# DataCTE/SDXL-Training-Improvements

Measured on AMD Instinct MI355X. Metric: images/sec/node SDXL-base 1024^2 bf16 fwd+bwd, higher is better.
Workload: dtype bf16; 1 GPU; method=ddpm v_prediction + zero_terminal_snr + MinSNR(5), SDXL-base UNet fwd+bwd, batch 4/GPU, 1024^2 (latent 128x128); global_batch=4, parallelism=dp1, weights=synthetic (counter-hash init of the 2,567,463,684-parameter SDXL-base UNet)

## Files before the change

sdxl-training-improvements_amd/csrc/gemm.hip:

```cpp
#include "gemm_tiles.h"

#include <stdio.h>
#include <stdlib.h>

#include <type_traits>
#include <vector>

#define BM 128
#ifndef GEMM_DIRECT_EPILOGUE
#define GEMM_DIRECT_EPILOGUE 1
#endif

static int g_mode256 = 1;
static int g_force_cfg = 0;
#ifdef SDXL_DIAG
static int g_sk_mode = 0;
#endif

static constexpr int cdiv_c(int a, int b) { return (a + b - 1) / b; }
__device__ unsigned g_ln_spin_error = 0;
__device__ __forceinline__ float row16_sum(float v) {
  v += __builtin_bit_cast(float, __builtin_amdgcn_update_dpp(0, __builtin_bit_cast(int, v), 0x111, 0xf, 0xf, true));
  v += __builtin_bit_cast(float, __builtin_amdgcn_update_dpp(0, __builtin_bit_cast(int, v), 0x112, 0xf, 0xf, true));
  v += __builtin_bit_cast(float, __builtin_amdgcn_update_dpp(0, __builtin_bit_cast(int, v), 0x114, 0xf, 0xf, true));
  v += __builtin_bit_cast(float, __builtin_amdgcn_update_dpp(0, __builtin_bit_cast(int, v), 0x118, 0xf, 0xf, true));
  return v;
}
__device__ __forceinline__ bf16x8 z8() {
  bf16x8 z;
#pragma unroll
  for (int e = 0; e < 8; ++e) z[e] = (bf16)0.f;
  return z;
}
static constexpr int gemm_smem_bytes(int BN, int S, int BK, int NW = 4) {
  const bool pad = ((BM * BK * 2 / 1024) % NW) != 0 || ((BN * BK * 2 / 1024) % NW) != 0;
  int ring = S * (BM + BN) * BK * 2 + (pad ? 1024 : 0), stg = BK == 32 ? 0 : 64 * (BN + 4) * 4;
  return ring > stg ? ring : stg;
}
static constexpr int gemm_occupancy(int BN, int S, int BK, int NW) {
  int byl = (160 * 1024) / gemm_smem_bytes(BN, S, BK, NW);
  return NW == 8 ? 1 : (byl > 3 ? 3 : (byl < 1 ? 1 : byl));
}

template <int FORM, bool CONV, int BN, int S, int BK, bool FAST, int NW, bool KSP = false, bool PL = false>
__global__ __launch_bounds__(NW * 64, PL ? 2 : gemm_occupancy(BN, S, BK, NW)) void gemm_kernel(const GemmP pin) {
  GemmP p = pin;
  set_wave_prio(pin.prio);
  int bx, by, bz = blockIdx.z, ztap = 0;
  if (FORM == GEMM_TN && pin.xcd_bh > 0) {
    const int tz = pin.group > 1 ? 1 : (int)gridDim.z / pin.splitk;
    xcd_seq_map(pin.xcd_bh, tz, bx, by, ztap, bz);
  } else xcd_tile_map(pin.xcd_px, bx, by);
  if (FORM == GEMM_TN && pin.group > 1) {
    const int gi = bz;
    p.A = pin.gA[gi]; p.B = pin.gB[gi]; p.C = pin.gC[gi]; p.bias_grad = pin.gbias_grad[gi]; p.Cb = pin.gCb[gi];
  }
  static_assert(!KSP || (NW == 8 && BK == 64 && FAST && S >= 3 && FORM != GEMM_TN), "split-K groups: 8 waves, BK 64, FAST staging, ring >= 3");
  static_assert(!PL || (NW == 4 && BK == 64 && FAST && S >= 3 && FORM != GEMM_TN && !KSP), "pipelined loop: 4 waves, BK 64, FAST staging, ring >= 3, NT / NN");
  constexpr int BMT = BM;
  constexpr int A_TILE_BYTES = BMT * BK * 2;
  constexpr int B_TILE_BYTES = BN * BK * 2;
  constexpr int STAGE_BYTES = A_TILE_BYTES + B_TILE_BYTES;
  constexpr int RING_BYTES = S * STAGE_BYTES;
  constexpr int WGM = KSP ? 2 : NW / 2;
  constexpr int MI = BMT / (WGM * 16);
  constexpr int NJ = BN / 32;
  constexpr int NCA = A_TILE_BYTES / 1024;
  constexpr int NCB = B_TILE_BYTES / 1024;
  constexpr int ACH = cdiv_c(NCA, NW);
  constexpr int BCH = cdiv_c(NCB, NW);
  constexpr int NL = ACH + BCH;
  constexpr int VR = BK / 8;
  constexpr int KC_ROWS = 64 / VR;
  constexpr int LDC = BN + 4;
  constexpr int NT = NW * 64;
  constexpr bool PIPE = true;
  constexpr bool DIRECT = GEMM_DIRECT_EPILOGUE;
  extern __shared__ __attribute__((aligned(16))) char smem[];
  const int tid = threadIdx.x;
  const int lane = tid & 63;
  const int wave = __builtin_amdgcn_readfirstlane(tid >> 6);
  const int kg = KSP ? wave >> 2 : 0;
  const int wm = KSP ? (wave >> 1) & 1 : wave >> 1, wn = wave & 1;
  const int l16 = lane & 15, g = lane >> 4;
#ifdef SDXL_GEMM_DIAG
  constexpr int dbg = SDXL_GEMM_DIAG;
#else
  constexpr int dbg = 0;
#endif
  const int n0 = (dbg & 8) ? 0 : bx * BN;
  const int m0 = (dbg & 8) ? 0 : by * BMT;

  int tap_fixed = 0, split = 0;
  if (FORM == GEMM_TN && p.group <= 1) {
    if (pin.xcd_bh > 0) {
      split = bz;
      tap_fixed = ztap;
    } else {
      tap_fixed = bz / p.splitk;
      split = bz - tap_fixed * p.splitk;
    }
  }
  constexpr bool NSPLIT = FORM != GEMM_TN && FAST && !KSP;
  if (NSPLIT && p.splitk > 1) split = bz;
  const int ktiles_per_tap = (p.K + BK - 1) / BK;
  int kt_begin = 0, kt_end;
  if (FORM == GEMM_TN) {
    int chunk = (ktiles_per_tap + p.splitk - 1) / p.splitk;
    kt_begin = split * chunk;
    kt_end = min(ktiles_per_tap, kt_begin + chunk);
  } else if (NSPLIT && p.splitk > 1) {
    const int total = ktiles_per_tap * p.taps;
    int chunk = (total + p.splitk - 1) / p.splitk;
    kt_begin = split * chunk;
    kt_end = min(total, kt_begin + chunk);
  } else {
    kt_end = ktiles_per_tap * p.taps;
  }
  const int dn_phase = (FORM == GEMM_NN && CONV && p.up2 == 2) ? m0 / p.up_plane : 0;
  const int dn_nb = (dn_phase & 1) ? 2 : 1;
  if (FORM == GEMM_NN && CONV && p.up2 == 2) kt_end = ktiles_per_tap * ((dn_phase >> 1) ? 2 : 1) * dn_nb;

  const int kc_rowl = lane / VR, kc_pv = lane % VR;
  PixRow arow[ACH];
  if (CONV && !FAST && FORM != GEMM_TN) {
#pragma unroll
    for (int j = 0; j < ACH; ++j) arow[j] = decode_pix(m0 + (wave + j * NW) * KC_ROWS + kc_rowl, p.M, p.Hm, p.Wm);
  }
  const bf16* zsrc = (const bf16*)g_zero16;
  char* const pad_dst = smem + RING_BYTES;

  constexpr bool CF = FAST && CONV;
  const bf16* pa[ACH];
  const bf16* pb[BCH];
  long sa[ACH], sb[BCH];
  int amask[ACH];
  int bok[BCH];
  int by_[BCH], bx_[BCH];
  long ua = 0, ub = 0;
  int s_tap = 0, s_c = 0;
  const int tdy = (SDXL_UP2_3 && p.up2 == 3) ? (tap_fixed / 3 == 0 ? -1 : 0) : p.up2 ? up2_dy(tap_fixed) : tap_fixed / 3 - 1;
  const int tdx = (SDXL_UP2_3 && p.up2 == 3) ? (tap_fixed % 3 == 0 ? -1 : 0) : p.up2 ? up2_dx(tap_fixed) : tap_fixed - (tap_fixed / 3) * 3 - 1;
  const long s3_plane = (SDXL_UP2_3 && p.up2 == 3) ? (long)(((tap_fixed / 3 != 1) ? 2 : 0) + ((tap_fixed % 3 != 1) ? 1 : 0)) * p.up_plane : 0;
  const int up_phase = (CF && FORM == GEMM_NT && p.up2) ? m0 / p.up_plane : dn_phase;
  auto tap_offsets = [&]() {
    int dy, dx, wtap;
    long plane = 0;
    if (FORM == GEMM_NT && (SDXL_UP2_3 && p.up2 == 3)) {
      const int ky = s_tap / 3, kx = s_tap - ky * 3;
      dy = ky == 0 ? -1 : 0; dx = kx == 0 ? -1 : 0;
      wtap = s_tap;
      plane = (long)((ky != 1 ? 2 : 0) + (kx != 1 ? 1 : 0)) * p.up_plane * p.lda;
    } else
    if (FORM == GEMM_NN && p.up2 == 2) {
      const int a = dn_phase >> 1, b = dn_phase & 1;
      const int ry = s_tap / dn_nb, rx = s_tap - ry * dn_nb;
      const int ky = a ? (ry == 0 ? 0 : 2) : 1, kx = b ? (rx == 0 ? 0 : 2) : 1;
      dy = a ? (ry == 0 ? 1 : 0) : 0; dx = b ? (rx == 0 ? 1 : 0) : 0;
      wtap = ky * 3 + kx;
    } else
    if (p.up2) {
      const int e = FORM == GEMM_NT ? up_phase * 4 + s_tap : s_tap;
      dy = up2_dy(e); dx = up2_dx(e); wtap = e;
// ... 130 lines not shown
  auto advance = [&]() {
    if (!CF) return;
    if (FORM == GEMM_TN) {
      ua += (long)BK * p.lda;
      ub += (long)BK * p.ldb;
      const int dxs = BK % p.Wm, dys = BK / p.Wm;
#pragma unroll
      for (int j = 0; j < BCH; ++j) {
        bx_[j] += dxs;
        if (bx_[j] >= p.Wm) { bx_[j] -= p.Wm; by_[j] += 1; }
        by_[j] += dys;
        if (by_[j] >= p.Hm) by_[j] -= p.Hm;
      }
    } else {
      if (++s_c == ktiles_per_tap) { s_c = 0; ++s_tap; }
      tap_offsets();
    }
  };
  bool dma_on = true;
  auto issue_piece = [&](int pc, int buf, bool live) {
    if (dbg && !dma_on) return;
    char* At = smem + buf * STAGE_BYTES;
    char* Bt = At + A_TILE_BYTES;
#pragma unroll
    for (int j = 0; j < ACH; ++j)
      if (pc == j) {
        const int c = wave + j * NW;
        const bf16* src;
        if (CF) {
          const bool v = live && (FORM == GEMM_TN ? amask[j] != 0 : ((amask[j] >> s_tap) & 1) != 0);
          src = v ? pa[j] + ua : zsrc;
        } else {
          src = live ? pa[j] : zsrc;
        }
        char* dst = (NCA % NW == 0 || c < NCA) ? At + c * 1024 : pad_dst;
        if (PL) lds_dma16_global(src, lds_addr_of(dst));
        else __builtin_amdgcn_global_load_lds((gbl_void*)src, (lds_void*)dst, 16, 0, 0);
        if (!CF) pa[j] += sa[j];
      }
#pragma unroll
    for (int j = 0; j < BCH; ++j)
      if (pc == ACH + j) {
        const int c = wave + j * NW;
        const bf16* src;
        if (CF) {
          bool v = live && bok[j] != 0;
          if (FORM == GEMM_TN) {
            const int ys = by_[j] + tdy, xs = bx_[j] + tdx;
            v = v && ys >= 0 && ys < p.Hm && xs >= 0 && xs < p.Wm;
          }
          src = v ? pb[j] + ub : zsrc;
        } else {
          src = live ? pb[j] : zsrc;
        }
        char* dst = (NCB % NW == 0 || c < NCB) ? Bt + c * 1024 : pad_dst;
        if (PL) lds_dma16_global(src, lds_addr_of(dst));
        else __builtin_amdgcn_global_load_lds((gbl_void*)src, (lds_void*)dst, 16, 0, 0);
        if (!CF) pb[j] += sb[j];
      }
  };

  auto stage_gen = [&](int kt, int buf) {
    int tap = 0, c0;
    if (FORM == GEMM_TN) {
      tap = tap_fixed;
      c0 = kt * BK;
    } else {
      tap = kt / ktiles_per_tap;
      c0 = (kt - tap * ktiles_per_tap) * BK;
    }
    const int dy = tap / 3, dx = tap - dy * 3;
    char* At = smem + buf * STAGE_BYTES;
    char* Bt = At + A_TILE_BYTES;
#pragma unroll
    for (int j = 0; j < ACH; ++j) {
      const int c = wave + j * NW;
      const bool cok = NCA % NW == 0 || c < NCA;
      const bf16* src;
      if (FORM == GEMM_TN) {
        const int krow = c * 4 + (lane >> 4);
        const int kk = c0 + krow;
        const int m = m0 + (nc_logical<128>(krow, lane & 15) << 3);
        src = (cok && kk < p.K && m < p.M) ? p.A + (long)kk * p.lda + m : zsrc;
      } else {
        const int row = c * KC_ROWS + kc_rowl;
        const int kofs = c0 + ((kc_pv ^ kc_swz<BK>(row)) << 3);
        if (CONV) {
          long s = gather_src(arow[j], dy, dx, p);
          src = (cok && s >= 0 && kofs < p.K) ? p.A + s * p.lda + kofs : zsrc;
        } else {
          const int m = m0 + row;
          src = (cok && m < p.M && kofs < p.K) ? p.A + (long)m * p.lda + kofs : zsrc;
        }
      }
      __builtin_amdgcn_global_load_lds((gbl_void*)src, (lds_void*)(cok ? At + c * 1024 : pad_dst), 16, 0, 0);
    }
#pragma unroll
    for (int j = 0; j < BCH; ++j) {
      const int c = wave + j * NW;
      const bool cok = NCB % NW == 0 || c < NCB;
      const bf16* src;
      if (FORM == GEMM_NT) {
        const int wtap = p.flip ? (p.taps - 1 - tap) : tap;
        const int row = c * KC_ROWS + kc_rowl;
        const int n = n0 + row;
        const int kofs = c0 + ((kc_pv ^ kc_swz<BK>(row)) << 3);
        src = (cok && n < p.N && kofs < p.K) ? p.B + (long)n * p.ldb + (long)wtap * p.b_tap_stride + kofs : zsrc;
      } else {
        constexpr int V = BN / 8;
        const int q = c * 64 + lane;
        const int krow = q / V, pv = q - krow * V;
        const int kk = c0 + krow;
        const int n = n0 + (nc_logical<BN>(krow, pv) << 3);
        if (FORM == GEMM_NN) {
          const int wtap = p.flip ? (p.taps - 1 - tap) : tap;
          src = (cok && kk < p.K && n < p.N) ? p.B + (long)kk * p.ldb + (long)wtap * p.b_tap_stride + n : zsrc;
        } else {
          long s;
          if (CONV) {
            PixRow r = decode_pix(kk, p.K, p.Hm, p.Wm);
            s = gather_src(r, dy, dx, p);
          } else {
            s = kk < p.K ? kk : -1;
          }
          src = (cok && s >= 0 && n < p.N) ? p.B + s * p.ldb + n : zsrc;
        }
      }
      __builtin_amdgcn_global_load_lds((gbl_void*)src, (lds_void*)(cok ? Bt + c * 1024 : pad_dst), 16, 0, 0);
    }
  };
  auto stage = [&](int kt, int buf) {
    if (FAST) {
#pragma unroll
      for (int pc = 0; pc < NL; ++pc) issue_piece(pc, buf, true);
      advance();
    } else {
      stage_gen(kt, buf);
    }
  };

  f32x4 acc[MI][NJ];
#pragma unroll
  for (int i = 0; i < MI; ++i)
#pragma unroll
    for (int j = 0; j < NJ; ++j) acc[i][j] = (f32x4){0.f, 0.f, 0.f, 0.f};
  const bool do_bias = FORM == GEMM_TN && p.bias_grad != nullptr && bx == 0 && (p.up2 == 1 ? (tap_fixed & 3) == 0 : tap_fixed == 0) && wn == 0;
  f32x4 accb[MI];
  bf16x8 ones;
#pragma unroll
  for (int i = 0; i < MI; ++i) accb[i] = (f32x4){0.f, 0.f, 0.f, 0.f};
#pragma unroll
  for (int e = 0; e < 8; ++e) ones[e] = (bf16)1.0f;

  const int T = kt_end - kt_begin;
  constexpr int U = 1;
#pragma unroll
  for (int d = 0; d < S - U; ++d) {
    if (d < T) stage(kt_begin + d, d);
    else if (FAST) {
#pragma unroll
      for (int pc = 0; pc < NL; ++pc) issue_piece(pc, d, false);
      advance();
    }
  }
  int rd = 0, wr = S - U;
  if (dbg & 2) dma_on = false;
  constexpr int KS = BK / 32;
  struct FragK { bf16x8 a[MI], b[NJ]; };
  auto read_ks = [&](int slot, int ks, FragK& f) {
    const char* At = smem + slot * STAGE_BYTES;
    const char* Bt = At + A_TILE_BYTES;
    if (dbg & 4) {
#pragma unroll
      for (int i = 0; i < MI; ++i) f.a[i] = ones;
#pragma unroll
      for (int j = 0; j < NJ; ++j) f.b[j] = ones;
      return;
    }
#pragma unroll
    for (int i = 0; i < MI; ++i) {
      if (FORM == GEMM_TN)
        f.a[i] = frag_nc<128>(At, ks * 32 + g * 8, wm * (MI * 16) + i * 16, l16);
      else
        f.a[i] = frag_kc<BK>(At, wm * (MI * 16) + i * 16 + l16, ks * 4 + g);
      if (i == 0) {
#pragma unroll
        for (int j = 0; j < NJ; ++j) {
          if (FORM == GEMM_NT)
            f.b[j] = frag_kc<BK>(Bt, wn * (BN / 2) + j * 16 + l16, ks * 4 + g);
          else
            f.b[j] = frag_nc<BN>(Bt, ks * 32 + g * 8, wn * (BN / 2) + j * 16, l16);
        }
      }
    }
  };
  auto mfma_ks = [&](const FragK& f, int ks, int wslot, bool live) {
    if (FORM == GEMM_TN && do_bias) {
#pragma unroll
      for (int i = 0; i < MI; ++i) accb[i] = __builtin_amdgcn_mfma_f32_16x16x32_bf16(f.a[i], ones, accb[i], 0, 0, 0);
    }
    if (!FAST) __builtin_amdgcn_s_setprio(1);
#pragma unroll
    for (int i = 0; i < MI; ++i) {
#pragma unroll
      for (int j = 0; j < NJ; ++j) {
        if (dbg & 1) acc[i][j][0] += (float)f.a[i][0] + (float)f.b[j][0];
        else if (DIRECT) acc[i][j] = __builtin_amdgcn_mfma_f32_16x16x32_bf16(f.b[j], f.a[i], acc[i][j], 0, 0, 0);
        else acc[i][j] = __builtin_amdgcn_mfma_f32_16x16x32_bf16(f.a[i], f.b[j], acc[i][j], 0, 0, 0);
      }
      if (FAST) {
        constexpr int NSLOT = KSP ? MI : KS * MI;
        const int slot = KSP ? i : ks * MI + i;
#pragma unroll
        for (int pc = 0; pc < NL; ++pc)
          if (pc % NSLOT == slot) issue_piece(pc, wslot, live);
      }
    }
    if (!FAST) __builtin_amdgcn_s_setprio(0);
  };
  if constexpr (PL) {
    constexpr int NG = MI;
    constexpr int NITEM = MI + NJ;
    constexpr int RG = 3;
    auto np0 = []() constexpr { int n = 0; for (int pc = 0; pc < NL; ++pc) if (pc % (2 * NG) < NG) ++n; return n; };
    auto read_item = [&](int slot, int ks, FragK& f, int it) {
      const char* At = smem + slot * STAGE_BYTES;
      const char* Bt = At + A_TILE_BYTES;
      if (dbg & 4) { if (it < NJ) f.b[it] = ones; else f.a[it - NJ] = ones; return; }
      if (it < NJ) {
        const int j = it;
        if (FORM == GEMM_NT) f.b[j] = frag_kc<BK>(Bt, wn * (BN / 2) + j * 16 + l16, ks * 4 + g);
        else f.b[j] = frag_nc<BN>(Bt, ks * 32 + g * 8, wn * (BN / 2) + j * 16, l16);
      } else {
        const int i = it - NJ;
        f.a[i] = frag_kc<BK>(At, wm * (MI * 16) + i * 16 + l16, ks * 4 + g);
      }
    };
    auto phase = [&](auto PHC, const FragK& fc, FragK& fn, int rslot, int rks, int wslot, bool live) {
      constexpr int PH = decltype(PHC)::value;
#pragma unroll
      for (int gi = 0; gi < NG; ++gi) {
#pragma unroll
        for (int j = 0; j < NJ; ++j) {
          if (dbg & 1) acc[gi][j][0] += (float)fc.a[gi][0] + (float)fc.b[j][0];
          else acc[gi][j] = __builtin_amdgcn_mfma_f32_16x16x32_bf16(fc.b[j], fc.a[gi], acc[gi][j], 0, 0, 0);
        }
        __builtin_amdgcn_sched_barrier(0);
        if (gi < RG) {
#pragma unroll
          for (int it = 0; it < NITEM; ++it)
            if (it * RG / NITEM == gi) read_item(rslot, rks, fn, it);
        }
#pragma unroll
        for (int pc = 0; pc < NL; ++pc)
          if (pc % (2 * NG) == PH * NG + gi) issue_piece(pc, wslot, live);
        __builtin_amdgcn_sched_barrier(0);
      }
    };
    FragK f0, f1;
    wait_vmcnt<(S - 2) * NL>();
    __builtin_amdgcn_s_barrier();
#pragma unroll
    for (int it = 0; it < NITEM; ++it) read_item(rd, 0, f0, it);
    for (int t = 0; t < T; ++t) {
      const bool live = t + S - 1 < T;
      phase(std::integral_constant<int, 0>{}, f0, f1, rd, 1, wr, live);
      wait_vmcnt<(S - 3) * NL + np0()>();
      asm volatile("s_waitcnt lgkmcnt(0)" ::: "memory");
      __builtin_amdgcn_sched_barrier(0);
      __builtin_amdgcn_s_barrier();
      const int rn = rd + 1 == S ? 0 : rd + 1;
      phase(std::integral_constant<int, 1>{}, f1, f0, rn, 0, wr, live);
      advance();
      rd = rn;
      wr = wr + 1 == S ? 0 : wr + 1;
    }
  } else
  if (KSP) {
    wait_vmcnt<(S - 2) * NL>();
    __builtin_amdgcn_s_barrier();
    if (kg == 1) __builtin_amdgcn_s_barrier();
    for (int t = 0; t < T; ++t) {
      FragK f;
      read_ks(rd, kg, f);
      wait_vmcnt<(S - 3) * NL>();
      __builtin_amdgcn_sched_barrier(0);
      __builtin_amdgcn_s_barrier();
      __builtin_amdgcn_s_setprio(1);
      mfma_ks(f, kg, wr, t + S - 1 < T);
      __builtin_amdgcn_s_setprio(0);
      advance();
      __builtin_amdgcn_sched_barrier(0);
      __builtin_amdgcn_s_barrier();
      rd = rd + 1 == S ? 0 : rd + 1;
      wr = wr + 1 == S ? 0 : wr + 1;
    }
    if (kg == 0) __builtin_amdgcn_s_barrier();
  } else
  for (int t = 0; t < T; ++t) {
    if (FAST) wait_vmcnt<(S - 2) * NL>();
    else if (S >= 3 && t + S - 2 < T) wait_vmcnt<(S - 2) * NL>();
    else wait_vmcnt<0>();
    __builtin_amdgcn_s_barrier();
    const bool live = t + S - 1 < T;
    if (!FAST && live) stage(kt_begin + t + S - 1, wr);
    FragK f[KS];
#pragma unroll
    for (int ks = 0; ks < KS; ++ks) read_ks(rd, ks, f[ks]);
    if (PIPE) __builtin_amdgcn_sched_barrier(0);
#pragma unroll
    for (int ks = 0; ks < KS; ++ks) mfma_ks(f[ks], ks, wr, live);
    if (FAST) advance();
    rd = rd + 1 == S ? 0 : rd + 1;
    wr = wr + 1 == S ? 0 : wr + 1;
  }
  wait_vmcnt<0>();
  if (KSP) {
    __syncthreads();
    float* X = (float*)smem;
#pragma unroll
    for (int i = 0; i < MI; ++i) {
      if ((i >> 1) == kg) continue;
#pragma unroll
      for (int j = 0; j < NJ; ++j)
        *(f32x4*)(X + (wm * 64 + i * 16 + l16) * LDC + wn * (BN / 2) + j * 16 + g * 4) = acc[i][j];
    }
    __syncthreads();
#pragma unroll
    for (int i = 0; i < MI; ++i) {
      if ((i >> 1) != kg) continue;
#pragma unroll
      for (int j = 0; j < NJ; ++j) {
        const f32x4 o = *(const f32x4*)(X + (wm * 64 + i * 16 + l16) * LDC + wn * (BN / 2) + j * 16 + g * 4);
        acc[i][j][0] += o[0]; acc[i][j][1] += o[1]; acc[i][j][2] += o[2]; acc[i][j][3] += o[3];
      }
    }
  }
  if (FORM == GEMM_TN && do_bias && l16 == 0) {
#pragma unroll
    for (int i = 0; i < MI; ++i)
#pragma unroll
      for (int r = 0; r < 4; ++r) {
        const int m = m0 + wm * (MI * 16) + i * 16 + g * 4 + r;
        if (m < p.M) {
          if (p.up2 == 1) atomicAdd(p.bias_grad + m, accb[i][r]);
          else gemm_bias_out(p.bias_grad, p.slab, p.slab_ld, p.splitk, split, p.M, m, accb[i][r]);
        }
      }
  }
  auto store_bf16 = [&](int m, int n, float (&x)[8], int cnt) {
    if (m >= p.M || n >= p.N) return;
    if (cnt == 8) {
      if (p.bias) {
        bf16x8 bv = *(const bf16x8*)(p.bias + n);
#pragma unroll
        for (int e = 0; e < 8; ++e) x[e] += (float)bv[e];
      }
      if (p.rowvec) {
        bf16x8 tv = *(const bf16x8*)(p.rowvec + (long)(m / p.rows_per_batch) * p.ldv + n);
#pragma unroll
        for (int e = 0; e < 8; ++e) x[e] += (float)tv[e];
      }
      if (p.resid) {
        bf16x8 rv = *(const bf16x8*)(p.resid + (long)m * p.ldr + n);
#pragma unroll
        for (int e = 0; e < 8; ++e) x[e] += (float)rv[e];
      }
      bf16x8 o;
#pragma unroll
      for (int e = 0; e < 8; ++e) o[e] = (bf16)x[e];
      *(bf16x8*)((bf16*)p.C + (long)m * p.ldc + n) = o;
    } else {
      if (p.bias) {
        bf16x4 bv = *(const bf16x4*)(p.bias + n);
#pragma unroll
        for (int e = 0; e < 4; ++e) x[e] += (float)bv[e];
      }
      if (p.rowvec) {
        bf16x4 tv = *(const bf16x4*)(p.rowvec + (long)(m / p.rows_per_batch) * p.ldv + n);
#pragma unroll
        for (int e = 0; e < 4; ++e) x[e] += (float)tv[e];
      }
      if (p.resid) {
        bf16x4 rv = *(const bf16x4*)(p.resid + (long)m * p.ldr + n);
#pragma unroll
        for (int e = 0; e < 4; ++e) x[e] += (float)rv[e];
      }
      bf16x4 o;
#pragma unroll
      for (int e = 0; e < 4; ++e) o[e] = (bf16)x[e];
      *(bf16x4*)((bf16*)p.C + (long)m * p.ldc + n) = o;
    }
  };
  if (NSPLIT && p.splitk > 1) {
#pragma unroll
    for (int i = 0; i < MI; ++i) {
      const int m = m0 + wm * (MI * 16) + i * 16 + l16;
      if (m >= p.M) continue;
#pragma unroll
      for (int j = 0; j < NJ; ++j) {
        const int n = n0 + wn * (BN / 2) + j * 16 + g * 4;
        if (n >= p.N) continue;
        *(f32x4*)(p.slab + ((long)split * p.M + m) * p.slab_ld + n) = acc[i][j];
      }
    }
    return;
  }
  constexpr bool LN_OK = SDXL_LN_EPILOGUE && FORM == GEMM_NN && !CONV && BN == 128 && NW == 4 && !KSP && FAST && BK == 64 && S == 2;
  if constexpr (LN_OK) if (p.ln_x) {
    constexpr int NP = NJ / 2;
    asm volatile("s_nop 7\n\ts_nop 7\n\ts_nop 7" ::: "memory");
    __syncthreads();
    float* rowpart = (float*)smem;
    float* rowtot = rowpart + 2 * 128 * 2;
    float* colpart = rowtot + 2 * 128 * 2;
    const int wcol = n0 + wn * (BN / 2);
    const int mrow = m0 + wm * (MI * 16) + l16;
    float s1[MI], s2[MI], mean[MI], rstd[MI];
#pragma unroll
    for (int i = 0; i < MI; ++i) {
      const bool mok = mrow + i * 16 < p.M;
      mean[i] = mok ? p.ln_stats[(long)(mrow + i * 16) * 2] : 0.f;
      rstd[i] = mok ? p.ln_stats[(long)(mrow + i * 16) * 2 + 1] : 0.f;
      s1[i] = 0.f; s2[i] = 0.f;
    }
#pragma unroll
    for (int jp = 0; jp < NP; ++jp) {
      const int j = 2 * jp;
      const int nc = wcol + (j + (g & 1)) * 16 + (g >> 1) * 8;
      const bool nok = nc < p.N;
      bf16x8 gv = z8();
      if (nok) gv = *(const bf16x8*)(p.ln_gamma + nc);
      float pg[8], pb[8];
#pragma unroll
      for (int e = 0; e < 8; ++e) { pg[e] = 0.f; pb[e] = 0.f; }
#pragma unroll
      for (int i = 0; i < MI; ++i) {
        const int m = mrow + i * 16;
        const bool ok = nok && m < p.M;
        float v[8];
#pragma unroll
        for (int r = 0; r < 4; ++r) {
          float lo = acc[i][j][r], hi = acc[i][j + 1][r];
          asm volatile("s_nop 1\n\tv_permlane16_swap_b32 %0, %1" : "+v"(lo), "+v"(hi));
          lo = (float)(bf16)lo; hi = (float)(bf16)hi;
          acc[i][j][r] = lo; acc[i][j + 1][r] = hi;
          v[r] = lo; v[4 + r] = hi;
        }
        if (p.C && ok) {
          bf16x8 o;
#pragma unroll
          for (int e = 0; e < 8; ++e) o[e] = (bf16)v[e];
          *(bf16x8*)((bf16*)p.C + (long)m * p.ldc + nc) = o;
        }
        bf16x8 xv = z8();
        if (ok) xv = *(const bf16x8*)(p.ln_x + (long)m * p.ln_ldx + nc);
#pragma unroll
        for (int e = 0; e < 8; ++e) {
          const float xh = ((float)xv[e] - mean[i]) * rstd[i];
          const float t = v[e] * (float)gv[e];
          s1[i] += t; s2[i] += t * xh;
          pg[e] += v[e] * xh; pb[e] += v[e];
        }
        __builtin_amdgcn_sched_barrier(0);
      }
      if (p.ln_pcol) {
#pragma unroll
        for (int e = 0; e < 8; ++e) {
// ... 45 lines not shown
    __syncthreads();
    if (tid == 0) __hip_atomic_store(flags + (long)bx * gridDim.y + by, (unsigned)p.ln_epoch, __ATOMIC_RELAXED, __HIP_MEMORY_SCOPE_AGENT);
    if (tid < 64) {
      int spins = 0;
      bool ok;
      do {
        unsigned f = (unsigned)p.ln_epoch;
        if (tid < ncolt) f = __hip_atomic_load(flags + (long)tid * gridDim.y + by, __ATOMIC_RELAXED, __HIP_MEMORY_SCOPE_AGENT);
        ok = __all(f == (unsigned)p.ln_epoch);
        if (!ok) __builtin_amdgcn_s_sleep(4);
      } while (!ok && ++spins < (1 << 22));
      if (!ok && tid == 0) atomicOr(&g_ln_spin_error, 1u);
    }
    __syncthreads();
    {
      constexpr int KC = 5;
      const int row = tid & (BMT - 1), h = tid >> 7;
      u64 a[KC], b[KC];
      int spins = 0;
      bool ok;
      do {
#pragma unroll
        for (int k = 0; k < KC; ++k) {
          const int c = 2 * k + h;
          a[k] = tag; b[k] = tag;
          if (c < ncolt) {
            const u64* src = slots + ((long)c * Mpad + m0 + row) * 2;
            a[k] = __hip_atomic_load(src, __ATOMIC_RELAXED, __HIP_MEMORY_SCOPE_AGENT);
            b[k] = __hip_atomic_load(src + 1, __ATOMIC_RELAXED, __HIP_MEMORY_SCOPE_AGENT);
          }
        }
        ok = true;
#pragma unroll
        for (int k = 0; k < KC; ++k) ok = ok && (a[k] >> 32) == (tag >> 32) && (b[k] >> 32) == (tag >> 32);
        if (!ok) __builtin_amdgcn_s_sleep(8);
      } while (!ok && ++spins < (1 << 20));
      if (!ok) atomicOr(&g_ln_spin_error, 2u);
      float S1 = 0.f, S2 = 0.f;
#pragma unroll
      for (int k = 0; k < KC; ++k)
        if (2 * k + h < ncolt) { S1 += __uint_as_float((unsigned)a[k]); S2 += __uint_as_float((unsigned)b[k]); }
      rowtot[(h * BMT + row) * 2] = S1;
      rowtot[(h * BMT + row) * 2 + 1] = S2;
    }
    __syncthreads();
    float S1[MI], S2[MI];
#pragma unroll
    for (int i = 0; i < MI; ++i) {
      const int row = wm * (MI * 16) + i * 16 + l16;
      const float invn = 1.f / (float)p.N;
      S1[i] = (rowtot[row * 2] + rowtot[(BMT + row) * 2]) * invn; S2[i] = (rowtot[row * 2 + 1] + rowtot[(BMT + row) * 2 + 1]) * invn;
    }
#pragma unroll
    for (int jp = 0; jp < NP; ++jp) {
      const int j = 2 * jp;
      const int nc = wcol + (j + (g & 1)) * 16 + (g >> 1) * 8;
      if (nc >= p.N) continue;
      const bf16x8 gv = *(const bf16x8*)(p.ln_gamma + nc);
#pragma unroll
      for (int i = 0; i < MI; ++i) {
        const int m = mrow + i * 16;
        if (m >= p.M) continue;
        const bf16x8 xv = *(const bf16x8*)(p.ln_x + (long)m * p.ln_ldx + nc);
        bf16x8 o;
        if (p.ln_addend) o = *(const bf16x8*)(p.ln_addend + (long)m * p.ln_ldo + nc);
#pragma unroll
        for (int e = 0; e < 8; ++e) {
          const float v = e < 4 ? acc[i][j][e & 3] : acc[i][j + 1][e & 3];
          const float xh = ((float)xv[e] - mean[i]) * rstd[i];
          float d = rstd[i] * (v * (float)gv[e] - S1[i] - xh * S2[i]);
          if (p.ln_addend) d += (float)o[e];
          o[e] = (bf16)d;
        }
        *(bf16x8*)(p.ln_dx + (long)m * p.ln_ldo + nc) = o;
        __builtin_amdgcn_sched_barrier(0);
      }
    }
    return;
  }
  if (FORM == GEMM_TN || !p.geglu) {
    if (FORM != GEMM_TN) asm volatile("s_nop 7\n\ts_nop 7\n\ts_nop 7" ::: "memory");
#pragma unroll
    for (int i = 0; i < MI; ++i) {
      if (KSP && (i >> 1) != kg) continue;
      const int m = m0 + wm * (MI * 16) + i * 16 + l16;
      if (FORM == GEMM_TN) {
        if (m >= p.M) continue;
#pragma unroll
        for (int j = 0; j < NJ; ++j) {
          const int n = n0 + wn * (BN / 2) + j * 16 + g * 4;
          if (n >= p.N) continue;
          f32x4 x = acc[i][j];
          float* c = (float*)p.C + (long)m * p.ldc + (long)tap_fixed * p.c_tap_stride + n;
          if (p.splitk > 1) {
            *(f32x4*)(p.slab + ((long)split * p.M + m) * p.slab_ld + (long)tap_fixed * p.c_tap_stride + n) = x;
          } else if (p.Cb) {
            if (p.accumulate) {
              const f32x4 a = *(const f32x4*)c;
              x[0] += a[0]; x[1] += a[1]; x[2] += a[2]; x[3] += a[3];
            }
            bf16x4 o;
            o[0] = (bf16)(x[0] * p.cb_scale); o[1] = (bf16)(x[1] * p.cb_scale);
            o[2] = (bf16)(x[2] * p.cb_scale); o[3] = (bf16)(x[3] * p.cb_scale);
            *(bf16x4*)(p.Cb + (long)m * p.ldc + (long)tap_fixed * p.c_tap_stride + n) = o;
          } else if (p.accumulate) {
            f32x4 a = *(f32x4*)c;
            a[0] += x[0]; a[1] += x[1]; a[2] += x[2]; a[3] += x[3];
            *(f32x4*)c = a;
          } else {
            *(f32x4*)c = x;
          }
        }
      } else {
        constexpr bool DELTA_OK = FORM == GEMM_NN && BN == 128 && NW == 4 && !KSP;
        float dl = 0.f;
#pragma unroll
        for (int j = 0; j + 1 < NJ; j += 2) {
          float x[8];
#pragma unroll
          for (int r = 0; r < 4; ++r) {
            float lo = acc[i][j][r], hi = acc[i][j + 1][r];
            asm volatile("s_nop 1\n\tv_permlane16_swap_b32 %0, %1" : "+v"(lo), "+v"(hi));
            x[r] = lo;
            x[4 + r] = hi;
          }
          const int n = n0 + wn * (BN / 2) + (j + (g & 1)) * 16 + (g >> 1) * 8;
          store_bf16(m, n, x, 8);
          if (DELTA_OK && p.delta_out && m < p.M && n < p.N) {
            const bf16x8 ov = *(const bf16x8*)(p.delta_o + (long)m * p.delta_ldo + n);
#pragma unroll
            for (int e = 0; e < 8; ++e) dl += (float)(bf16)x[e] * (float)ov[e];
          }
        }
        if (DELTA_OK && p.delta_out) {
          float a = dl, b2 = dl;
          asm volatile("s_nop 1\n\tv_permlane16_swap_b32 %0, %1" : "+v"(a), "+v"(b2));
          dl = a + b2;
          a = dl; b2 = dl;
          asm volatile("s_nop 1\n\tv_permlane32_swap_b32 %0, %1" : "+v"(a), "+v"(b2));
          dl = a + b2;
          if (g == 0 && m < p.M) {
            const int bb = m / p.delta_nq, qq = m - bb * p.delta_nq, hh = (n0 + wn * (BN / 2)) >> 6;
            if (hh < p.delta_heads) p.delta_out[((long)bb * p.delta_heads + hh) * p.delta_nq + qq] = dl;
          }
        }
        if (NJ & 1) {
          float x[8];
#pragma unroll
          for (int r = 0; r < 4; ++r) x[r] = acc[i][NJ - 1][r];
          store_bf16(m, n0 + wn * (BN / 2) + (NJ - 1) * 16 + g * 4, x, 4);
        }
      }
    }
    return;
  }
  __syncthreads();
  float* Cs = (float*)smem;
  constexpr int VPR = BN / 8;
#pragma unroll 1
  for (int half = 0; half < BMT / 64; ++half) {
    const int wrow = wm * (MI * 16);
    if (wrow / 64 == half) {
#pragma unroll
      for (int i = 0; i < MI; ++i) {
        if (KSP && (i >> 1) != kg) continue;
#pragma unroll
        for (int j = 0; j < NJ; ++j)
          *(f32x4*)(Cs + (wrow - half * 64 + i * 16 + l16) * LDC + wn * (BN / 2) + j * 16 + g * 4) = acc[i][j];
      }
    }
    __syncthreads();
    if (FORM != GEMM_TN && (BN == 128 || BN == 160)) {
      constexpr int G = BN / 2;
      for (int id = tid; id < 64 * VPR; id += NT) {
        const int row = id / VPR, col = (id - row * VPR) * 8;
        const int m = m0 + half * 64 + row;
        if (m >= p.M) continue;
        if (FORM == GEMM_NT) {
          if (col >= G || n0 + col >= p.N) continue;
          const int na = n0 + col, nt = na + G;
          float xa[8], xt[8];
#pragma unroll
          for (int e = 0; e < 8; ++e) { xa[e] = Cs[row * LDC + col + e]; xt[e] = Cs[row * LDC + G + col + e]; }
          if (p.bias) {
            bf16x8 ba = *(const bf16x8*)(p.bias + na), bt = *(const bf16x8*)(p.bias + nt);
#pragma unroll
            for (int e = 0; e < 8; ++e) { xa[e] += (float)ba[e]; xt[e] += (float)bt[e]; }
          }
          bf16x8 oa, ot, og;
#pragma unroll
          for (int e = 0; e < 8; ++e) {
            oa[e] = (bf16)xa[e];
            ot[e] = (bf16)xt[e];
            og[e] = (bf16)((float)oa[e] * gelu_f((float)ot[e]));
          }
          *(bf16x8*)((bf16*)p.C + (long)m * p.ldc + na) = oa;
          *(bf16x8*)((bf16*)p.C + (long)m * p.ldc + nt) = ot;
          *(bf16x8*)(p.aux + (long)m * p.ldaux + (n0 >> 1) + col) = og;
        } else {
          const int n = n0 + col;
          if (n >= p.N) continue;
          const int Gp = p.geglu_group;
          const long cu = (long)(n / Gp) * (2 * Gp) + (n % Gp);
          bf16x8 ua = *(const bf16x8*)(p.aux + (long)m * p.ldaux + cu);
          bf16x8 ut = *(const bf16x8*)(p.aux + (long)m * p.ldaux + cu + Gp);
          bf16x8 oa, ot;
#pragma unroll
          for (int e = 0; e < 8; ++e) {
            const float dv = (float)(bf16)Cs[row * LDC + col + e], tv = (float)ut[e];
            float cdf, pdf;
            gelu_cdf_pdf(tv, &cdf, &pdf);
            oa[e] = (bf16)(dv * tv * cdf);
            ot[e] = (bf16)(dv * (float)ua[e] * fmaf(tv, pdf, cdf));
          }
          *(bf16x8*)((bf16*)p.C + (long)m * p.ldc + cu) = oa;
          *(bf16x8*)((bf16*)p.C + (long)m * p.ldc + cu + Gp) = ot;
        }
      }
    }
    __syncthreads();
  }
}

__global__ void splitk_reduce_kernel(const float* __restrict__ slab, float* __restrict__ C, int M, int cols, long ldc,
                                     long slab_ld, int splitk, int accumulate, bf16* __restrict__ Cb, float cb_scale,
                                     float* __restrict__ bias_grad) {
  const int vpr = cols / 4;
  for (long i = (long)blockIdx.x * blockDim.x + threadIdx.x; i < (long)M * vpr; i += (long)gridDim.x * blockDim.x) {
    long m = i / vpr;
    int c = (int)(i - m * vpr) * 4;
    if (bias_grad && c == 0) {
      const float* tail = slab + (long)splitk * M * slab_ld + m;
      float b = 0.f;
      for (int s = 0; s < splitk; ++s) b += tail[(long)s * M];
      bias_grad[m] += b;
    }
    f32x4 a = accumulate ? *(const f32x4*)(C + m * ldc + c) : (f32x4){0.f, 0.f, 0.f, 0.f};
    for (int s = 0; s < splitk; ++s) {
      f32x4 v = *(const f32x4*)(slab + ((long)s * M + m) * slab_ld + c);
      a[0] += v[0]; a[1] += v[1]; a[2] += v[2]; a[3] += v[3];
    }
    if (Cb) {
      bf16x4 o;
      o[0] = (bf16)(a[0] * cb_scale); o[1] = (bf16)(a[1] * cb_scale); o[2] = (bf16)(a[2] * cb_scale); o[3] = (bf16)(a[3] * cb_scale);
      *(bf16x4*)(Cb + m * ldc + c) = o;
    } else {
      *(f32x4*)(C + m * ldc + c) = a;
    }
  }
}

__global__ void splitk_epilogue_kernel(const float* __restrict__ slab, bf16* __restrict__ C, int M, int N, long ldc, long slab_ld,
                                       int splitk, const bf16* __restrict__ bias, const bf16* __restrict__ resid, long ldr,
                                       const bf16* __restrict__ rowvec, long ldv, int rows_per_batch) {
  const int vpr = N / 8;
  for (long i = (long)blockIdx.x * blockDim.x + threadIdx.x; i < (long)M * vpr; i += (long)gridDim.x * blockDim.x) {
    const long m = i / vpr;
    const int n = (int)(i - m * vpr) * 8;
    float x[8] = {0.f, 0.f, 0.f, 0.f, 0.f, 0.f, 0.f, 0.f};
    for (int s = 0; s < splitk; ++s) {
      const float* sp = slab + ((long)s * M + m) * slab_ld + n;
      const f32x4 a = *(const f32x4*)sp, b = *(const f32x4*)(sp + 4);
      x[0] += a[0]; x[1] += a[1]; x[2] += a[2]; x[3] += a[3]; x[4] += b[0]; x[5] += b[1]; x[6] += b[2]; x[7] += b[3];
    }
    if (bias) {
      const bf16x8 v = *(const bf16x8*)(bias + n);
#pragma unroll
      for (int e = 0; e < 8; ++e) x[e] += (float)v[e];
    }
    if (rowvec) {
      const bf16x8 v = *(const bf16x8*)(rowvec + (m / rows_per_batch) * ldv + n);
#pragma unroll
      for (int e = 0; e < 8; ++e) x[e] += (float)v[e];
    }
    if (resid) {
      const bf16x8 v = *(const bf16x8*)(resid + m * ldr + n);
#pragma unroll
      for (int e = 0; e < 8; ++e) x[e] += (float)v[e];
    }
    bf16x8 o;
#pragma unroll
    for (int e = 0; e < 8; ++e) o[e] = (bf16)x[e];
    *(bf16x8*)(C + m * ldc + n) = o;
  }
}

int gemm_ln_cfg(int M, int N, int K) {
  if (K % 64 || N % 8 || M <= 0) return 0;
  const long t128 = (long)cdiv(M, BM) * cdiv(N, 128);
  return t128 <= 512 && cdiv(N, 128) <= 10 ? 1 : 0;
}
size_t gemm_ln_part_floats(int M, int N) {
  return (size_t)cdiv(N, 128) * cdiv(M, BM) * BM * 4 + (size_t)cdiv(N, 128) * cdiv(M, BM) + 4;
}
size_t gemm_ln_pcol_floats(int M, int N) { return (size_t)cdiv(M, BM) * 2 * N; }
int gemm_ln_rowblocks(int M) { return cdiv(M, BM); }

#ifdef SDXL_DIAG
int gemm_ln_error(unsigned* out) {
  HIP_CHECK_RET(hipDeviceSynchronize());
  HIP_CHECK_RET(hipMemcpyFromSymbol(out, HIP_SYMBOL(g_ln_spin_error), sizeof(unsigned)));
  const unsigned z = 0;
  HIP_CHECK_RET(hipMemcpyToSymbol(HIP_SYMBOL(g_ln_spin_error), &z, sizeof(unsigned)));
  return 0;
}
#endif
// ... 534 lines not shown
```

Before: 37.42 images/sec.

## Add specialized GEGLU dgrad epilogue with prefetched aux loads in last k-step

Adds a dedicated epilogue for the NN GEMM when geglu==2. It stages the accumulator as bf16 in shared memory and computes both GEGLU input gradients (gate and value) directly, writing them to their interleaved column positions. The aux activation loads are issued during the final k-iteration, around the MFMAs, so their latency overlaps compute instead of stalling the epilogue. In exchange it raises register pressure from holding the prefetched vectors and adds a separate specialized main-loop path.

```diff
diff --git a/sdxl-training-improvements_amd/csrc/gemm.hip b/sdxl-training-improvements_amd/csrc/gemm.hip
--- a/sdxl-training-improvements_amd/csrc/gemm.hip
+++ b/sdxl-training-improvements_amd/csrc/gemm.hip
@@ -9,6 +9,9 @@
 #define BM 128
 #ifndef GEMM_DIRECT_EPILOGUE
 #define GEMM_DIRECT_EPILOGUE 1
+#endif
+#ifndef GEMM_GEGLU_PREFETCH
+#define GEMM_GEGLU_PREFETCH 1
 #endif
 
 static int g_mode256 = 1;
@@ -445,6 +448,38 @@
 #pragma unroll
   for (int e = 0; e < 8; ++e) ones[e] = (bf16)1.0f;
 
+  constexpr bool G2B = FORM == GEMM_NN && !CONV && NW == 4 && !KSP && !PL && FAST && S == 2 && BK == 64 && (BN == 128 || BN == 160);
+  constexpr bool G2PF = G2B && GEMM_GEGLU_PREFETCH;
+  constexpr int G2V = BN / 8;
+  constexpr int G2H = G2B ? 64 * G2V / NT : 1;
+  static_assert(!G2B || (64 * G2V) % NT == 0, "GEGLU dgrad epilogue: whole ids per thread and half");
+  const bool g2 = G2B && p.geglu == 2;
+  unsigned g2off[G2H];
+  unsigned g2ok = 0;
+  bf16x8 ua0[G2H], ut0[G2H], ua1[G2H], ut1[G2H];
+  if (G2B && g2) {
+#pragma unroll
+    for (int k = 0; k < G2H; ++k) {
+      const int id = tid + k * NT, row = id / G2V;
+      const int n = n0 + (id % G2V) * 8;
+      const int Gp = p.geglu_group;
+      const int cu = (n / Gp) * (2 * Gp) + (n % Gp);
+      const bool ok = n < p.N && m0 + row < p.M;
+      if (ok) g2ok |= 1u << k;
+      if (n < p.N && m0 + 64 + row < p.M) g2ok |= 256u << k;
+      g2off[k] = ok ? (unsigned)(row * (int)p.ldaux + cu) * 2u : 0u;
+      ua0[k] = z8(); ut0[k] = z8(); ua1[k] = z8(); ut1[k] = z8();
+    }
+  }
+  auto g2_load = [&](int half, int k, bf16x8& va, bf16x8& vt) {
+    const char* b = (const char*)(p.aux + (long)m0 * p.ldaux);
+    if (half && m0 + 64 < p.M) b += 128L * p.ldaux;
+    unsigned o = (half == 0 || ((g2ok >> (8 + k)) & 1)) ? g2off[k] : 0u;
+    asm volatile("" : "+v"(o));
+    va = *(const bf16x8*)(b + o);
+    vt = *(const bf16x8*)(b + 2L * p.geglu_group + o);
+  };
+
   const int T = kt_end - kt_begin;
   constexpr int U = 1;
 #pragma unroll
@@ -590,23 +625,60 @@
     }
     if (kg == 0) __builtin_amdgcn_s_barrier();
   } else
-  for (int t = 0; t < T; ++t) {
-    if (FAST) wait_vmcnt<(S - 2) * NL>();
-    else if (S >= 3 && t + S - 2 < T) wait_vmcnt<(S - 2) * NL>();
-    else wait_vmcnt<0>();
-    __builtin_amdgcn_s_barrier();
-    const bool live = t + S - 1 < T;
-    if (!FAST && live) stage(kt_begin + t + S - 1, wr);
-    FragK f[KS];
-#pragma unroll
-    for (int ks = 0; ks < KS; ++ks) read_ks(rd, ks, f[ks]);
-    if (PIPE) __builtin_amdgcn_sched_barrier(0);
-#pragma unroll
-    for (int ks = 0; ks < KS; ++ks) mfma_ks(f[ks], ks, wr, live);
-    if (FAST) advance();
-    rd = rd + 1 == S ? 0 : rd + 1;
-    wr = wr + 1 == S ? 0 : wr + 1;
-  }
+  {
+    bool g2_looped = false;
+    if constexpr (G2PF) if (g2) {
+      auto kstep = [&](int t, auto G2LASTC) {
+        constexpr bool G2LAST = decltype(G2LASTC)::value;
+        wait_vmcnt<(S - 2) * NL>();
+        __builtin_amdgcn_s_barrier();
+        const bool live = t + S - 1 < T;
+        FragK f[KS];
+#pragma unroll
+        for (int ks = 0; ks < KS; ++ks) read_ks(rd, ks, f[ks]);
+        __builtin_amdgcn_sched_barrier(0);
+        if (G2LAST) {
+#pragma unroll
+          for (int k = 0; k < G2H; ++k) g2_load(0, k, ua0[k], ut0[k]);
+          __builtin_amdgcn_sched_barrier(0);
+        }
+#pragma unroll
+        for (int ks = 0; ks < KS; ++ks) mfma_ks(f[ks], ks, wr, live);
+        if (G2LAST) {
+          __builtin_amdgcn_sched_barrier(0);
+#pragma unroll
+          for (int k = 0; k < G2H; ++k) g2_load(1, k, ua1[k], ut1[k]);
+          __builtin_amdgcn_sched_barrier(0);
+        }
+        advance();
+        rd = rd + 1 == S ? 0 : rd + 1;
+        wr = wr + 1 == S ? 0 : wr + 1;
+      };
+      for (int t = 0; t < T - 1; ++t) kstep(t, std::false_type{});
+      kstep(T - 1, std::true_type{});
+      g2_looped = true;
+    }
+    if (!g2_looped)
+    for (int t = 0; t < T; ++t) {
+      if (FAST) wait_vmcnt<(S - 2) * NL>();
+      else if (S >= 3 && t + S - 2 < T) wait_vmcnt<(S - 2) * NL>();
+      else wait_vmcnt<0>();
+      __builtin_amdgcn_s_barrier();
+      const bool live = t + S - 1 < T;
+      if (!FAST && live) stage(kt_begin + t + S - 1, wr);
+      FragK f[KS];
+#pragma unroll
+      for (int ks = 0; ks < KS; ++ks) read_ks(rd, ks, f[ks]);
+      if (PIPE) __builtin_amdgcn_sched_barrier(0);
+#pragma unroll
+      for (int ks = 0; ks < KS; ++ks) mfma_ks(f[ks], ks, wr, live);
+      if (FAST) advance();
+      rd = rd + 1 == S ? 0 : rd + 1;
+      wr = wr + 1 == S ? 0 : wr + 1;
+    }
+  }
+  if (G2PF && g2) wait_vmcnt<2 * G2H>();
+  else
   wait_vmcnt<0>();
   if (KSP) {
     __syncthreads();
@@ -958,6 +1030,64 @@
         }
       }
     }
+    return;
+  }
+  if constexpr (G2B) if (g2) {
+    auto g2_pin = [](bf16x8& v) {
+      typedef unsigned u32x4 __attribute__((ext_vector_type(4)));
+      u32x4 r = __builtin_bit_cast(u32x4, v);
+      asm volatile("" : "+v"(r));
+      v = __builtin_bit_cast(bf16x8, r);
+    };
+    if (!G2PF) {
+#pragma unroll
+      for (int k = 0; k < G2H; ++k) g2_load(0, k, ua0[k], ut0[k]);
+#pragma unroll
+      for (int k = 0; k < G2H; ++k) g2_load(1, k, ua1[k], ut1[k]);
+    }
+    constexpr int LDB = BN + 8;
+    bf16* Cb = (bf16*)smem;
+    __builtin_amdgcn_sched_barrier(0);
+    __builtin_amdgcn_s_barrier();
+#pragma unroll
+    for (int i = 0; i < MI; ++i)
+#pragma unroll
+      for (int j = 0; j < NJ; ++j) {
+        bf16x4 o;
+#pragma unroll
+        for (int r = 0; r < 4; ++r) o[r] = (bf16)acc[i][j][r];
+        *(bf16x4*)(Cb + (wm * (MI * 16) + i * 16 + l16) * LDB + wn * (BN / 2) + j * 16 + g * 4) = o;
+      }
+    asm volatile("s_waitcnt lgkmcnt(0)" ::: "memory");
+    __builtin_amdgcn_sched_barrier(0);
+    __builtin_amdgcn_s_barrier();
+    const int Gp = p.geglu_group;
+#pragma unroll
+    for (int half = 0; half < 2; ++half)
+#pragma unroll
+      for (int k = 0; k < G2H; ++k) {
+        const int id = tid + k * NT;
+        const int row = half * 64 + id / G2V, col = (id % G2V) * 8;
+        const int m = m0 + row;
+        const bool ok = (g2ok >> (half * 8 + k)) & 1;
+        const bf16x8 dg = *(const bf16x8*)(Cb + row * LDB + col);
+        const bf16x8 ua = half ? ua1[k] : ua0[k], ut = half ? ut1[k] : ut0[k];
+        bf16x8 oa, ot;
+#pragma unroll
+        for (int e = 0; e < 8; ++e) {
+          const float dv = (float)dg[e], tv = (float)ut[e];
+          float cdf, pdf;
+          gelu_cdf_pdf(tv, &cdf, &pdf);
+          oa[e] = (bf16)(dv * tv * cdf);
+          ot[e] = (bf16)(dv * (float)ua[e] * fmaf(tv, pdf, cdf));
+        }
+        g2_pin(oa); g2_pin(ot);
+        if (ok) {
+          const int cu = (int)(g2off[k] >> 1) - (id / G2V) * (int)p.ldaux;
+          *(bf16x8*)((bf16*)p.C + (long)m * p.ldc + cu) = oa;
+          *(bf16x8*)((bf16*)p.C + (long)m * p.ldc + cu + Gp) = ot;
+        }
+      }
     return;
   }
   __syncthreads();
```

After: 37.59 images/sec, median of 6. About the same (+0.4%).
